# ZYM-PKU/UDiffText

Measured on AMD Instinct MI355X. Metric: 512x512 50-step denoised images/sec (UDiffText hot path: conditioner + 50 CFG Euler steps + VAE decode), higher is better.
Workload: dtype bf16; 1 GPU; 512x512, 50 Euler/DDIM(eta 0) steps, CFG 5.0, 9-char labels, noise_iters 0; global batch 4 per step sharded over 1 GPU(s) = 4 images per GPU in micro-batches of 4: every UNet call runs ONE batch of 4 (8 samples with CFG); 3 such batch(es) in flight per GPU on separate launch streams; BASELINE.json configs[1]; global_batch=4, weights=synthetic (name-keyed recipe), 1361.2 M parameters, launch=hipGraph replay of the sampler steps, in_flight=3, batches_per_unet_call=1

## Files before the change

udifftext_amd/csrc/wide.h:

```cpp
#pragma once
#include <type_traits>

namespace wd {

using g8::buf_lds16;
using g8::OOB;
using g8::wait_vm;
using lg::C3Params;
using lg::raw_barrier;
using lg::wait_vm_upto;
using lg::wave_colstats;

struct WGeo {
  static constexpr int TW = 16, TH = 16, NW = 4;
  static constexpr int TM = 2, TN = 5, BN = TN * 32;
  static constexpr int PW = TW + 2, PH = TH + 2, PROWS = PW * PH;
  static constexpr int PIECES = (PROWS + 7) / 8;
  static constexpr int PATCH_BYTES = PIECES * 1024;
  static constexpr int W_BYTES = BN * ROW_BYTES;
  static constexpr int NRING = 3;
  static constexpr int RING = NRING * W_BYTES + 2 * PATCH_BYTES;
  static constexpr int EROW = BN * 4;
  static constexpr int STAGING = NW * 32 * EROW;
  static constexpr int SMEM = RING > STAGING ? RING : STAGING;
  static_assert(SMEM <= 160 * 1024, "one workgroup per CU");
};

template <bool STATS, bool PHASE = false>
__global__ void __launch_bounds__(256, 1) wconv3_kernel(const C3Params p) {
  using G = WGeo;
  constexpr int NT = PHASE ? 4 : 9;
  constexpr int NW = G::NW, TM = G::TM, TN = G::TN, BN = G::BN, PW = G::PW, NR = G::NRING;
  constexpr int WP = (BN / 8) / NW;
  constexpr int PP = (G::PIECES + NW - 1) / NW;
  constexpr int EROW = G::EROW;
  static_assert((BN / 8) % NW == 0, "weight pieces split evenly over the waves");
  extern __shared__ __attribute__((aligned(16))) char smem[];
  char* const wring = smem;
  char* const patches = smem + NR * G::W_BYTES;

  const int tid = threadIdx.x;
  const int wave = __builtin_amdgcn_readfirstlane(tid >> 6);
  const int lane = tid & 63;
  const int l31 = lane & 31;
  const int hi = lane >> 5;
  const int l3 = lane >> 3;
  const int pslot = lane & 7;
  const int row0 = wave * (TM * 32);
  const int swz_w = (l31 >> 1) & 7;
  const int w_frag_row = l31 * ROW_BYTES;

  const int unit = range_index(blockIdx.x, p.G);
  if (unit >= p.tiles * p.splitk * (PHASE ? 4 : 1)) return;
  const int phase = PHASE ? unit / (p.tiles * p.splitk) : 0;
  const int pha = phase >> 1, phb = phase & 1;
  const int ptile = unit / p.splitk;
  const int slice = unit - ptile * p.splitk;
  const int tile = ptile - phase * p.tiles;
  int tile_m, n0;
  {
    const int per_block = p.tiles_m * p.n_block;
    const int blk = tile / per_block;
    const int r = tile - blk * per_block;
    int nbw = p.tiles_n - blk * p.n_block;
    if (nbw > p.n_block) nbw = p.n_block;
    tile_m = r / nbw;
    n0 = (blk * p.n_block + (r - tile_m * nbw)) * BN;
  }
  const int per_img = p.tiles_x * p.tiles_y;
  const int b = tile_m / per_img;
  const int rt = tile_m - b * per_img;
  const int ty = rt / p.tiles_x;
  const int y0 = ty * G::TH, x0 = (rt - ty * p.tiles_x) * G::TW;
  const int c0 = slice * p.ch_per;
  int c1 = c0 + p.ch_per;
  if (c1 > p.chunks) c1 = p.chunks;

  const __amdgpu_buffer_rsrc_t rsrc_a = __builtin_amdgcn_make_buffer_rsrc(const_cast<uint16_t*>(p.a), 0, p.a_bytes, 0x00020000);
  const __amdgpu_buffer_rsrc_t rsrc_w =
      __builtin_amdgcn_make_buffer_rsrc(const_cast<uint16_t*>(p.w) + (PHASE ? (long long)phase * p.w_phase : 0LL), 0, p.w_bytes, 0x00020000);
  auto patch_swz = [](int prow, int yy) { return ((prow - 2 * yy) >> 1) & 7; };
  unsigned w_voff[WP], p_voff[PP];
  int p_piece[PP];
#pragma unroll
  for (int i = 0; i < WP; ++i) {
    const int row = (wave + NW * i) * 8 + l3;
    const int kw = (pslot ^ ((row >> 1) & 7)) * 8;
    const int n = n0 + row;
    w_voff[i] = (n < p.N) ? (unsigned)(((long long)n * p.ldw + kw) * 2) : OOB;
  }
#pragma unroll
  for (int i = 0; i < PP; ++i) {
    int idx = wave + NW * i;
    while (idx >= G::PIECES) idx -= NW;
    p_piece[i] = idx;
    const int prow = idx * 8 + l3;
    const int yy = prow / PW;
    const int xx = prow - yy * PW;
    const int gy = y0 + yy - 1, gx = x0 + xx - 1;
    const bool ok = (prow < G::PROWS) && ((unsigned)gy < (unsigned)p.H) && ((unsigned)gx < (unsigned)p.W);
    const int koff = (pslot ^ patch_swz(prow, yy)) * 8;
    p_voff[i] = ok ? (unsigned)(((((long long)b * p.H + gy) * p.W + gx) * p.C + koff) * 2) : OOB;
  }
  int a_prow[TM], a_py[TM];
#pragma unroll
  for (int tm = 0; tm < TM; ++tm) {
    const int ml = row0 + tm * 32 + l31;
    const int py = ml / G::TW, px = ml - py * G::TW;
    a_py[tm] = PHASE ? py + pha : py;
    a_prow[tm] = PHASE ? (py + pha) * PW + px + phb : py * PW + px;
  }
  auto issue_w = [&](int st, int c, int tap) {
    const int soff = (tap * p.C + c * 64) * 2;
    char* wbuf = wring + st * G::W_BYTES;
#pragma unroll
    for (int i = 0; i < WP; ++i) buf_lds16(rsrc_w, wbuf + (wave + NW * i) * 1024, w_voff[i], soff);
  };
  auto issue_patch = [&](int buf, int c) {
    char* pbuf = patches + buf * G::PATCH_BYTES;
#pragma unroll
    for (int i = 0; i < PP; ++i) buf_lds16(rsrc_a, pbuf + p_piece[i] * 1024, p_voff[i], c * 128);
  };

  f32x16 acc[TM][TN];
#pragma unroll
  for (int i = 0; i < TM; ++i)
#pragma unroll
    for (int j = 0; j < TN; ++j)
#pragma unroll
      for (int r = 0; r < 16; ++r) acc[i][j][r] = 0.f;

  constexpr int PPT = PHASE ? 6 : 2, PTAPS = (PP + PPT - 1) / PPT;
  static_assert(PTAPS <= NT - 2, "the next patch is complete two taps before its chunk starts");
  static_assert(NR - 1 < NT, "the ring's prologue stays inside the first chunk");
  auto issue_patch_part = [&](int buf, int c, int part) {
    char* pbuf = patches + buf * G::PATCH_BYTES;
#pragma unroll
    for (int j = 0; j < PPT; ++j) {
      const int i = part * PPT + j;
      if (i < PP) buf_lds16(rsrc_a, pbuf + p_piece[i] * 1024, p_voff[i], c * 128);
    }
  };
  issue_patch(c0 & 1, c0);
#pragma unroll
  for (int j = 0; j < NR - 1; ++j) issue_w(j, c0, j);
  int st = 0;
  for (int c = c0; c < c1; ++c) {
    const int cn = (c + 1 < c1) ? c + 1 : c;
    const char* pbuf = patches + (c & 1) * G::PATCH_BYTES;
    auto tap_body = [&](auto tap_c) {
      constexpr int tap = decltype(tap_c)::value;
      constexpr auto pcount = [](int t) { const int tt = (t + NT) % NT; return tt < PTAPS ? ((tt + 1) * PPT <= PP ? PPT : PP - tt * PPT) : 0; };
      wait_vm<pcount(tap - 2) + WP + pcount(tap - 1)>();
      raw_barrier();
      const int dy = PHASE ? tap >> 1 : tap / 3, dx = PHASE ? tap & 1 : tap - dy * 3;
      const char* wbuf = wring + st * G::W_BYTES;
      int arow[TM], aswz[TM];
#pragma unroll
      for (int t = 0; t < TM; ++t) {
        const int prow = a_prow[t] + dy * PW + dx;
        arow[t] = prow * ROW_BYTES;
        aswz[t] = patch_swz(prow, a_py[t] + dy);
      }
      bf16x8_t fx[2][TM], fw[2][TN];
      auto read_ks = [&](int ks, int slot2) {
        if (UDT_DBG(p.dbg, 3)) return;
#pragma unroll
        for (int t = 0; t < TM; ++t) fx[slot2][t] = lds_read_frag(pbuf + arow[t] + (((ks * 2 + hi) ^ aswz[t]) << 4));
        const int slot = ((ks * 2 + hi) ^ swz_w) << 4;
#pragma unroll
        for (int t = 0; t < TN; ++t) fw[slot2][t] = lds_read_frag(wbuf + w_frag_row + t * 32 * ROW_BYTES + slot);
      };
      read_ks(0, 0);
#pragma unroll
      for (int ks = 0; ks < 4; ++ks) {
        if (ks + 1 < 4) read_ks(ks + 1, (ks + 1) & 1);
        if (ks == 3) {
          const int ahead = tap + NR - 1;
          int s2 = st + NR - 1;
          if (s2 >= NR) s2 -= NR;
          if (!UDT_DBG(p.dbg, 0)) {
            if (ahead < NT) issue_w(s2, c, ahead);
            else issue_w(s2, cn, ahead - NT);
          }
          if constexpr (tap < PTAPS) {
            if (!UDT_DBG(p.dbg, 1)) issue_patch_part((c + 1) & 1, cn, tap);
          }
        }
        if (UDT_DBG(p.dbg, 2)) {
#pragma unroll
          for (int tm = 0; tm < TM; ++tm) asm volatile("" ::"v"(fx[ks & 1][tm]));
#pragma unroll
          for (int tn = 0; tn < TN; ++tn) asm volatile("" ::"v"(fw[ks & 1][tn]));
        } else {
#pragma unroll
          for (int tm = 0; tm < TM; ++tm)
#pragma unroll
            for (int tn = 0; tn < TN; ++tn) acc[tm][tn] = mfma32(fw[ks & 1][tn], fx[ks & 1][tm], acc[tm][tn]);
        }
      }
      __builtin_amdgcn_sched_group_barrier(0x100, TM + TN, 0);
#pragma unroll
      for (int ks = 0; ks < 3; ++ks) {
#pragma unroll
        for (int i = 0; i < TM + TN; ++i) {
          __builtin_amdgcn_sched_group_barrier(0x008, 1, 0);
          __builtin_amdgcn_sched_group_barrier(0x100, 1, 0);
        }
        __builtin_amdgcn_sched_group_barrier(0x008, TM * TN - (TM + TN), 0);
      }
      constexpr int NV = WP + pcount(tap), NVI = NV < TM * TN ? NV : TM * TN;
#pragma unroll
      for (int i = 0; i < NVI; ++i) {
        __builtin_amdgcn_sched_group_barrier(0x008, 1, 0);
        __builtin_amdgcn_sched_group_barrier(0x020, 1, 0);
      }
      if constexpr (NV > NVI) __builtin_amdgcn_sched_group_barrier(0x020, NV - NVI, 0);
      else __builtin_amdgcn_sched_group_barrier(0x008, TM * TN - NV, 0);
      st = (st + 1 == NR) ? 0 : st + 1;
    };
    tap_body(std::integral_constant<int, 0>{}); tap_body(std::integral_constant<int, 1>{}); tap_body(std::integral_constant<int, 2>{});
    tap_body(std::integral_constant<int, 3>{});
    if constexpr (!PHASE) {
      tap_body(std::integral_constant<int, 4>{}); tap_body(std::integral_constant<int, 5>{});
      tap_body(std::integral_constant<int, 6>{}); tap_body(std::integral_constant<int, 7>{}); tap_body(std::integral_constant<int, 8>{});
    }
  }
  constexpr int CPR = TN * 4;
  constexpr int RPI = 64 / CPR;
  constexpr int NIT = (32 + RPI - 1) / RPI;
  const int rl = lane / CPR;
  const int c8 = lane - rl * CPR;
  const int n = n0 + c8 * 8;
  const bool col_ok = (rl < RPI) && (n < p.N);
  long long mrow[TM][NIT];
  bool rok[TM][NIT];
  u32x4 rv[TM][NIT];
#pragma unroll
  for (int tm = 0; tm < TM; ++tm)
#pragma unroll
    for (int i = 0; i < NIT; ++i) {
      const int row = i * RPI + rl;
      rok[tm][i] = col_ok && row < 32;
      const int ml = row0 + tm * 32 + (row < 32 ? row : 0);
      const int py = ml / G::TW, px = ml - py * G::TW;
      mrow[tm][i] = PHASE ? ((long long)b * (2 * p.H) + (2 * (y0 + py) + pha)) * (2 * p.W) + (2 * (x0 + px) + phb)
                          : ((long long)b * p.H + (y0 + py)) * p.W + (x0 + px);
      u32x4 z = {0u, 0u, 0u, 0u};
      rv[tm][i] = z;
      if (p.res && rok[tm][i]) rv[tm][i] = *reinterpret_cast<const u32x4*>(p.res + mrow[tm][i] * p.ldr + n);
    }
  wait_vm<0>();
  raw_barrier();

  if (p.splitk > 1) {
    f32x4* slab = reinterpret_cast<f32x4*>(p.slabs + (long long)unit * (G::TW * G::TH * BN));
#pragma unroll
    for (int tm = 0; tm < TM; ++tm)
#pragma unroll
      for (int tn = 0; tn < TN; ++tn)
#pragma unroll
        for (int q = 0; q < 4; ++q) {
          f32x4 v = {acc[tm][tn][q * 4 + 0], acc[tm][tn][q * 4 + 1], acc[tm][tn][q * 4 + 2], acc[tm][tn][q * 4 + 3]};
          store16_sc1(slab + ((tm * TN + tn) * 4 + q) * 256 + tid, v);
        }
    asm volatile("s_waitcnt vmcnt(0)" ::: "memory");
    __syncthreads();
    int* const bcast = reinterpret_cast<int*>(smem);
    if (tid == 0) {
      const int t = __hip_atomic_fetch_add(p.counters + ptile, 1, __ATOMIC_RELAXED, __HIP_MEMORY_SCOPE_AGENT);
      const int last = (t == p.splitk - 1) ? 1 : 0;
      if (last) {
        __builtin_amdgcn_fence(__ATOMIC_ACQUIRE, "agent");
        __hip_atomic_store(p.counters + ptile, 0, __ATOMIC_RELAXED, __HIP_MEMORY_SCOPE_AGENT);
      }
      *bcast = last;
    }
    __syncthreads();
    const bool last = *bcast != 0;
    __syncthreads();
    if (!last) return;
#pragma unroll
    for (int i = 0; i < TM; ++i)
#pragma unroll
      for (int j = 0; j < TN; ++j)
#pragma unroll
        for (int r = 0; r < 16; ++r) acc[i][j][r] = 0.f;
    for (int s = 0; s < p.splitk; ++s) {
      const f32x4* sl = reinterpret_cast<const f32x4*>(p.slabs + ((long long)ptile * p.splitk + s) * (G::TW * G::TH * BN));
#pragma unroll
      for (int tm = 0; tm < TM; ++tm)
#pragma unroll
        for (int tn = 0; tn < TN; ++tn)
#pragma unroll
          for (int q = 0; q < 4; ++q) {
            const f32x4 v = sl[((tm * TN + tn) * 4 + q) * 256 + tid];
#pragma unroll
            for (int r = 0; r < 4; ++r) acc[tm][tn][q * 4 + r] += v[r];
          }
    }
  }

  char* const wl = smem + wave * (32 * EROW);
  f32x4 b0 = {0.f, 0.f, 0.f, 0.f}, b1 = b0;
  if (col_ok) {
    if (p.bias) {
      b0 = *reinterpret_cast<const f32x4*>(p.bias + n);
      b1 = *reinterpret_cast<const f32x4*>(p.bias + n + 4);
    }
    if (p.rowvec) {
      const float* rvp = p.rowvec + (long long)b * p.ldrv + n;
      const f32x4 r0 = *reinterpret_cast<const f32x4*>(rvp), r1 = *reinterpret_cast<const f32x4*>(rvp + 4);
#pragma unroll
      for (int j = 0; j < 4; ++j) b0[j] += r0[j], b1[j] += r1[j];
    }
  }
  float cs[8], cq[8];
#pragma unroll
  for (int j = 0; j < 8; ++j) cs[j] = cq[j] = 0.f;
#pragma unroll
  for (int tm = 0; tm < TM; ++tm) {
    {
      const int row = l31;
#pragma unroll
      for (int tn = 0; tn < TN; ++tn)
#pragma unroll
        for (int q = 0; q < 4; ++q) {
          const int chunk = (tn * 8 + q * 2 + hi) ^ (row & 7);
          f32x4 v = {acc[tm][tn][q * 4 + 0], acc[tm][tn][q * 4 + 1], acc[tm][tn][q * 4 + 2], acc[tm][tn][q * 4 + 3]};
          *reinterpret_cast<f32x4*>(wl + row * EROW + chunk * 16) = v;
        }
    }
#pragma unroll
    for (int i = 0; i < NIT; ++i) {
      const int row = i * RPI + rl;
      const int rr = row < 32 ? row : 0;
      const char* rp = wl + rr * EROW;
      const int sw = rr & 7;
      const f32x4 v0 = *reinterpret_cast<const f32x4*>(rp + (((2 * c8) ^ sw) << 4));
      const f32x4 v1 = *reinterpret_cast<const f32x4*>(rp + (((2 * c8 + 1) ^ sw) << 4));
      float o[8];
#pragma unroll
      for (int j = 0; j < 4; ++j) {
        o[j] = v0[j] * p.alpha + b0[j];
        o[4 + j] = v1[j] * p.alpha + b1[j];
      }
      if (p.res) {
#pragma unroll
        for (int j = 0; j < 4; ++j) {
          o[2 * j] += bf16_lo(rv[tm][i][j]);
          o[2 * j + 1] += bf16_hi(rv[tm][i][j]);
        }
      }
      if (rok[tm][i]) {
        u32x4 pk = {pack_bf16x2(o[0], o[1]), pack_bf16x2(o[2], o[3]), pack_bf16x2(o[4], o[5]), pack_bf16x2(o[6], o[7])};
        *reinterpret_cast<u32x4*>(p.out + mrow[tm][i] * p.ldo + n) = pk;
        if constexpr (STATS) {
#pragma unroll
          for (int j = 0; j < 4; ++j) {
            const float a = bf16_lo(pk[j]), bb = bf16_hi(pk[j]);
            cs[2 * j] += a; cq[2 * j] += a * a;
            cs[2 * j + 1] += bb; cq[2 * j + 1] += bb * bb;
          }
        }
      }
    }
  }
  if constexpr (STATS) {
    const int slot = (PHASE ? (b * 4 + phase) * per_img + rt : tile_m) * NW + wave;
    wave_colstats<CPR, RPI>(wl, lane, cs, cq, p.colstats + ((long long)slot * p.N + n) * 2, col_ok);
  }
}

}
```

Before: 10.94 images/s.

## Stream conv residual and bias vectors into LDS through the async load pipeline

The wide 3x3 conv kernel now prefetches bias and row-vector data into a small LDS area at kernel start. In the last K chunk it reuses the spare patch buffer to async-load half of the residual rows, replacing the epilogue's direct global loads. The first weight tile is issued earlier and the patch double-buffer parity is flipped so the final chunk's free buffer can hold the residual. This hides epilogue global-load latency behind the MMA loop, at the cost of more LDS, extra index registers and tighter ordering invariants between buffers.

Result: no change. 10.93 images/s (-0.1%).

```diff
diff --git a/udifftext_amd/csrc/wide.h b/udifftext_amd/csrc/wide.h
--- a/udifftext_amd/csrc/wide.h
+++ b/udifftext_amd/csrc/wide.h
@@ -22,7 +22,12 @@
   static constexpr int RING = NRING * W_BYTES + 2 * PATCH_BYTES;
   static constexpr int EROW = BN * 4;
   static constexpr int STAGING = NW * 32 * EROW;
-  static constexpr int SMEM = RING > STAGING ? RING : STAGING;
+  static constexpr int RP = 32 * BN * 2 / 1024;
+  static constexpr int RES_OFF = NRING * W_BYTES + PATCH_BYTES;
+  static_assert((32 * BN * 2) % 1024 == 0 && (NW * RP + 1) * 1024 <= PATCH_BYTES, "first-pass residual rows + filler fit a patch buffer");
+  static_assert(STAGING <= RES_OFF, "the staging blocks stay clear of the residual rows");
+  static constexpr int VEC_OFF = RING > STAGING ? RING : STAGING;
+  static constexpr int SMEM = VEC_OFF + 2 * 1024;
   static_assert(SMEM <= 160 * 1024, "one workgroup per CU");
 };
 
@@ -82,6 +87,15 @@
   auto patch_swz = [](int prow, int yy) { return ((prow - 2 * yy) >> 1) & 7; };
   unsigned w_voff[WP], p_voff[PP];
   int p_piece[PP];
+  char* const vecs = smem + G::VEC_OFF;
+  {
+    const int nv = n0 + lane * 4;
+    const unsigned v_voff = (lane * 4 < BN && nv < p.N) ? (unsigned)(nv * 4) : OOB;
+    if (wave == 0 && p.bias)
+      buf_lds16(__builtin_amdgcn_make_buffer_rsrc(const_cast<float*>(p.bias), 0, p.N * 4, 0x00020000), vecs, v_voff, 0);
+    if (wave == 1 && p.rowvec)
+      buf_lds16(__builtin_amdgcn_make_buffer_rsrc(const_cast<float*>(p.rowvec + (long long)b * p.ldrv), 0, p.N * 4, 0x00020000), vecs + 1024, v_voff, 0);
+  }
 #pragma unroll
   for (int i = 0; i < WP; ++i) {
     const int row = (wave + NW * i) * 8 + l3;
@@ -89,6 +103,14 @@
     const int n = n0 + row;
     w_voff[i] = (n < p.N) ? (unsigned)(((long long)n * p.ldw + kw) * 2) : OOB;
   }
+  auto issue_w = [&](int st, int c, int tap) {
+    const int soff = (tap * p.C + c * 64) * 2;
+    char* wbuf = wring + st * G::W_BYTES;
+#pragma unroll
+    for (int i = 0; i < WP; ++i) buf_lds16(rsrc_w, wbuf + (wave + NW * i) * 1024, w_voff[i], soff);
+  };
+  static_assert(NR == 3, "prologue: W(0), the first patch, W(1)");
+  issue_w(0, c0, 0);
 #pragma unroll
   for (int i = 0; i < PP; ++i) {
     int idx = wave + NW * i;
@@ -110,12 +132,13 @@
     a_py[tm] = PHASE ? py + pha : py;
     a_prow[tm] = PHASE ? (py + pha) * PW + px + phb : py * PW + px;
   }
-  auto issue_w = [&](int st, int c, int tap) {
-    const int soff = (tap * p.C + c * 64) * 2;
-    char* wbuf = wring + st * G::W_BYTES;
-#pragma unroll
-    for (int i = 0; i < WP; ++i) buf_lds16(rsrc_w, wbuf + (wave + NW * i) * 1024, w_voff[i], soff);
-  };
+  constexpr int RP = G::RP, SX = PHASE ? 2 : 1;
+  const bool res_loop = p.res != nullptr && p.splitk == 1;
+  const long long m_org = PHASE ? ((long long)b * (2 * p.H) + (2 * y0 + pha)) * (2 * p.W) + (2 * x0 + phb) : ((long long)b * p.H + y0) * p.W + x0;
+  const __amdgpu_buffer_rsrc_t rsrc_r =
+      __builtin_amdgcn_make_buffer_rsrc(const_cast<uint16_t*>(p.res ? p.res + m_org * p.ldr + n0 : p.a), 0, (int)OOB, 0x00020000);
+  unsigned r_voff[PP];
+  char* const resbuf = smem + G::RES_OFF;
   auto issue_patch = [&](int buf, int c) {
     char* pbuf = patches + buf * G::PATCH_BYTES;
 #pragma unroll
@@ -133,21 +156,34 @@
   constexpr int PPT = PHASE ? 6 : 2, PTAPS = (PP + PPT - 1) / PPT;
   static_assert(PTAPS <= NT - 2, "the next patch is complete two taps before its chunk starts");
   static_assert(NR - 1 < NT, "the ring's prologue stays inside the first chunk");
-  auto issue_patch_part = [&](int buf, int c, int part) {
+  auto issue_patch_part = [&](int buf, int c, bool res, int part) {
     char* pbuf = patches + buf * G::PATCH_BYTES;
+    const __amdgpu_buffer_rsrc_t rs = res ? rsrc_r : rsrc_a;
+    const int soff = res ? 0 : c * 128;
 #pragma unroll
     for (int j = 0; j < PPT; ++j) {
       const int i = part * PPT + j;
-      if (i < PP) buf_lds16(rsrc_a, pbuf + p_piece[i] * 1024, p_voff[i], c * 128);
+      if (i < PP) buf_lds16(rs, pbuf + (res ? (i < RP ? wave * RP + i : NW * RP) : p_piece[i]) * 1024, res ? r_voff[i] : p_voff[i], soff);
     }
   };
-  issue_patch(c0 & 1, c0);
-#pragma unroll
-  for (int j = 0; j < NR - 1; ++j) issue_w(j, c0, j);
+  issue_patch((c1 - 1 - c0) & 1, c0);
+  issue_w(1, c0, 1);
+#pragma unroll
+  for (int i = 0; i < PP; ++i) {
+    const int g16 = i * 64 + lane;
+    const int row = g16 / (BN / 8), cg = g16 - row * (BN / 8);
+    const int ml = row0 + row;
+    const int py = ml / G::TW, px = ml - py * G::TW;
+    const bool ok = i < RP && n0 + cg * 8 < p.N;
+    r_voff[i] = ok ? (unsigned)((((long long)(SX * py) * (SX * p.W) + SX * px) * p.ldr + cg * 8) * 2) : OOB;
+  }
   int st = 0;
   for (int c = c0; c < c1; ++c) {
-    const int cn = (c + 1 < c1) ? c + 1 : c;
-    const char* pbuf = patches + (c & 1) * G::PATCH_BYTES;
+    const bool tail = c + 1 >= c1;
+    const int cn = tail ? c : c + 1;
+    const bool res_now = tail && res_loop;
+    const int pb = (c1 - 1 - c) & 1;
+    const char* pbuf = patches + pb * G::PATCH_BYTES;
     auto tap_body = [&](auto tap_c) {
       constexpr int tap = decltype(tap_c)::value;
       constexpr auto pcount = [](int t) { const int tt = (t + NT) % NT; return tt < PTAPS ? ((tt + 1) * PPT <= PP ? PPT : PP - tt * PPT) : 0; };
@@ -184,7 +220,7 @@
             else issue_w(s2, cn, ahead - NT);
           }
           if constexpr (tap < PTAPS) {
-            if (!UDT_DBG(p.dbg, 1)) issue_patch_part((c + 1) & 1, cn, tap);
+            if (res_now || !UDT_DBG(p.dbg, 1)) issue_patch_part(pb ^ 1, cn, res_now, tap);
           }
         }
         if (UDT_DBG(p.dbg, 2)) {
@@ -233,9 +269,9 @@
   const int c8 = lane - rl * CPR;
   const int n = n0 + c8 * 8;
   const bool col_ok = (rl < RPI) && (n < p.N);
+  static_assert(TM == 2, "the first pass takes its residual rows from LDS, the second from registers");
   long long mrow[TM][NIT];
   bool rok[TM][NIT];
-  u32x4 rv[TM][NIT];
 #pragma unroll
   for (int tm = 0; tm < TM; ++tm)
 #pragma unroll
@@ -246,9 +282,6 @@
       const int py = ml / G::TW, px = ml - py * G::TW;
       mrow[tm][i] = PHASE ? ((long long)b * (2 * p.H) + (2 * (y0 + py) + pha)) * (2 * p.W) + (2 * (x0 + px) + phb)
                           : ((long long)b * p.H + (y0 + py)) * p.W + (x0 + px);
-      u32x4 z = {0u, 0u, 0u, 0u};
-      rv[tm][i] = z;
-      if (p.res && rok[tm][i]) rv[tm][i] = *reinterpret_cast<const u32x4*>(p.res + mrow[tm][i] * p.ldr + n);
     }
   wait_vm<0>();
   raw_barrier();
@@ -280,6 +313,10 @@
     const bool last = *bcast != 0;
     __syncthreads();
     if (!last) return;
+    if (p.res) {
+#pragma unroll
+      for (int i = 0; i < RP; ++i) buf_lds16(rsrc_r, resbuf + (wave * RP + i) * 1024, r_voff[i], 0);
+    }
 #pragma unroll
     for (int i = 0; i < TM; ++i)
 #pragma unroll
@@ -299,18 +336,26 @@
             for (int r = 0; r < 4; ++r) acc[tm][tn][q * 4 + r] += v[r];
           }
     }
+    wait_vm<0>();
+  }
+  u32x4 rv[NIT];
+#pragma unroll
+  for (int i = 0; i < NIT; ++i) {
+    u32x4 z = {0u, 0u, 0u, 0u};
+    rv[i] = z;
+    if (p.res && rok[1][i]) rv[i] = *reinterpret_cast<const u32x4*>(p.res + mrow[1][i] * p.ldr + n);
   }
 
   char* const wl = smem + wave * (32 * EROW);
   f32x4 b0 = {0.f, 0.f, 0.f, 0.f}, b1 = b0;
   if (col_ok) {
     if (p.bias) {
-      b0 = *reinterpret_cast<const f32x4*>(p.bias + n);
-      b1 = *reinterpret_cast<const f32x4*>(p.bias + n + 4);
+      b0 = *reinterpret_cast<const f32x4*>(vecs + c8 * 32);
+      b1 = *reinterpret_cast<const f32x4*>(vecs + c8 * 32 + 16);
     }
     if (p.rowvec) {
-      const float* rvp = p.rowvec + (long long)b * p.ldrv + n;
-      const f32x4 r0 = *reinterpret_cast<const f32x4*>(rvp), r1 = *reinterpret_cast<const f32x4*>(rvp + 4);
+      const char* rvp = vecs + 1024 + c8 * 32;
+      const f32x4 r0 = *reinterpret_cast<const f32x4*>(rvp), r1 = *reinterpret_cast<const f32x4*>(rvp + 16);
 #pragma unroll
       for (int j = 0; j < 4; ++j) b0[j] += r0[j], b1[j] += r1[j];
     }
@@ -346,10 +391,11 @@
         o[4 + j] = v1[j] * p.alpha + b1[j];
       }
       if (p.res) {
+        const u32x4 r = tm == 0 ? *reinterpret_cast<const u32x4*>(resbuf + wave * (RP * 1024) + i * (CPR * RPI * 16) + lane * 16) : rv[i];
 #pragma unroll
         for (int j = 0; j < 4; ++j) {
-          o[2 * j] += bf16_lo(rv[tm][i][j]);
-          o[2 * j + 1] += bf16_hi(rv[tm][i][j]);
+          o[2 * j] += bf16_lo(r[j]);
+          o[2 * j + 1] += bf16_hi(r[j]);
         }
       }
       if (rok[tm][i]) {
```
